# pennucci/PulsePortraiture

Measured on AMD Instinct MI355X. Metric: subint_fits_per_sec, higher is better.
Workload: dtype f64

## Files before the change

pulseportraiture_amd/csrc/pp_common.h:

```cpp
#pragma once
#include <hip/hip_runtime.h>
#include <stdint.h>
#include <type_traits>

namespace pp {

#define PP_DCONST 4149.377593360996
#define PP_TWO_PI 6.283185307179586476925286766559
#define PP_LN10 2.302585092994045684017991454684

typedef double2 cplx;

__device__ __forceinline__ cplx cmul(cplx a, cplx b) {
    return make_double2(fma(a.x, b.x, -a.y * b.y), fma(a.x, b.y, a.y * b.x));
}
__device__ __forceinline__ cplx cmulc(cplx a, cplx b) {
    return make_double2(fma(a.x, b.x, a.y * b.y), fma(a.y, b.x, -a.x * b.y));
}
__device__ __forceinline__ cplx cadd(cplx a, cplx b) { return make_double2(a.x + b.x, a.y + b.y); }
__device__ __forceinline__ cplx csub(cplx a, cplx b) { return make_double2(a.x - b.x, a.y - b.y); }
__device__ __forceinline__ cplx cmul_mi(cplx a) { return make_double2(a.y, -a.x); }
__device__ __forceinline__ double cnorm(cplx a) { return fma(a.x, a.x, a.y * a.y); }

template <typename T>
__device__ __forceinline__ const T* as_global(const T* p) {
    typedef const T __attribute__((address_space(1)))* gp_t;
    return (const T*)(gp_t)(uintptr_t)p;
}

template <typename T>
__device__ __forceinline__ T load_uniform(const T* p) {
    typedef const T __attribute__((address_space(4)))* cp_t;
    return *(cp_t)(uintptr_t)p;
}

__device__ __forceinline__ double rn_pin(double r) { asm volatile("" : "+v"(r)); return r; }
__device__ __forceinline__ double mul_rn(double a, double b) { return rn_pin(a * b); }
__device__ __forceinline__ double add_rn(double a, double b) { return rn_pin(a + b); }
__device__ __forceinline__ double sub_rn(double a, double b) { return rn_pin(a - b); }

__device__ __forceinline__ double recip_ge1(double x) {
    double y = __builtin_amdgcn_rcp(x);
    y = fma(fma(-x, y, 1.0), y, y);
    y = fma(fma(-x, y, 1.0), y, y);
    return (x < 1e300) ? y : 0.0;
}

template <bool SC>
__device__ __forceinline__ double kconst(double v) {
    if (SC) asm volatile("" : "+s"(v));
    return v;
}
template <bool SC = false>
__device__ __forceinline__ void sincos_turns(double t, double* sn, double* cs) {
    const double q = rint(4.0 * t);
    const double y = fma(-0.25, q, t);
    const double u = y * y;
    double ps = kconst<SC>(0x1.aaec32af93359p-4);
    ps = fma(ps, u, kconst<SC>(-0x1.6fadb9f155744p-1));
    ps = fma(ps, u, kconst<SC>(0x1.e8f434d018d63p+1));
    ps = fma(ps, u, kconst<SC>(-0x1.e3074fde8871fp+3));
    ps = fma(ps, u, kconst<SC>(0x1.50783487ee782p+5));
    ps = fma(ps, u, kconst<SC>(-0x1.32d2cce62bd86p+6));
    ps = fma(ps, u, kconst<SC>(0x1.466bc6775aae2p+6));
    ps = fma(ps, u, kconst<SC>(-0x1.4abbce625be53p+5));
    ps = fma(ps, u, kconst<SC>(0x1.921fb54442d18p+2));
    const double s0 = ps * y;
    double pc = kconst<SC>(0x1.20c62c2f2d7f5p-2);
    pc = fma(pc, u, kconst<SC>(-0x1.b6e24f44b128fp+0));
    pc = fma(pc, u, kconst<SC>(0x1.f9d38a3763cc3p+2));
    pc = fma(pc, u, kconst<SC>(-0x1.a6d1f2a204a8cp+4));
    pc = fma(pc, u, kconst<SC>(0x1.e1f506891babbp+5));
    pc = fma(pc, u, kconst<SC>(-0x1.55d3c7e3cbffap+6));
    pc = fma(pc, u, kconst<SC>(0x1.03c1f081b5ac4p+6));
    pc = fma(pc, u, kconst<SC>(-0x1.3bd3cc9be45dep+4));
    const double c0 = fma(pc, u, 1.0);
    const int qi = (int)q;
    const bool odd = qi & 1;
    const double so = odd ? c0 : s0, co = odd ? s0 : c0;
    *sn = (qi & 2) ? -so : so;
    *cs = ((qi + 1) & 2) ? -co : co;
}

template <bool SC = false>
__device__ __forceinline__ cplx unit_phasor(double k, double phi) {
    double pfrac = phi - rint(phi);
    double prod = k * pfrac;
    double err = fma(k, pfrac, -prod);
    double r = (prod - rint(prod)) + err;
    double s, c;
    sincos_turns<SC>(r, &s, &c);
    return make_double2(c, s);
}

template <int W>
__device__ __forceinline__ double group_sum(double v) {
#pragma unroll
    for (int o = W / 2; o > 0; o >>= 1) v += __shfl_xor(v, o, 64);
    return v;
}
template <int W>
__device__ __forceinline__ double group_max(double v) {
#pragma unroll
    for (int o = W / 2; o > 0; o >>= 1) v = fmax(v, __shfl_xor(v, o, 64));
    return v;
}

__device__ __forceinline__ int wave_reduce16_index(int lane) { return (lane >> 2) & 15; }
template <int NS>
__device__ __forceinline__ double wave_reduce16(const double (&s)[NS], int lane) {
    double t8[8], t4[4], t2[2];
    const bool b5 = lane & 32, b4 = lane & 16, b3 = lane & 8, b2 = lane & 4;
#pragma unroll
    for (int j = 0; j < 8; ++j) {
        const double hi = (j + 8 < NS) ? s[j + 8] : 0.0;
        const double keep = b5 ? hi : s[j], send = b5 ? s[j] : hi;
        t8[j] = keep + __shfl_xor(send, 32, 64);
    }
#pragma unroll
    for (int j = 0; j < 4; ++j) {
        const double keep = b4 ? t8[j + 4] : t8[j], send = b4 ? t8[j] : t8[j + 4];
        t4[j] = keep + __shfl_xor(send, 16, 64);
    }
#pragma unroll
    for (int j = 0; j < 2; ++j) {
        const double keep = b3 ? t4[j + 2] : t4[j], send = b3 ? t4[j] : t4[j + 2];
        t2[j] = keep + __shfl_xor(send, 8, 64);
    }
    const double keep = b2 ? t2[1] : t2[0], send = b2 ? t2[0] : t2[1];
    double v = keep + __shfl_xor(send, 4, 64);
    v += __shfl_xor(v, 2, 64);
    v += __shfl_xor(v, 1, 64);
    return v;
}

template <int NS>
__device__ __forceinline__ double wave_reduce_lds(const double (&s)[NS], int lane, double* buf) {
    static_assert(NS <= 16, "one value per lane quad");
    const int wpos = (lane >> 4) * 17 + (lane & 15);
#pragma unroll
    for (int q = 0; q < NS; ++q) buf[q * 68 + wpos] = s[q];
    const int q = min(lane >> 2, NS - 1), part = lane & 3;
    const double* src = buf + q * 68 + part * 17;
    double v = 0.0;
#pragma unroll
    for (int t = 0; t < 16; ++t) v += src[t];
    v += __shfl_xor(v, 1, 64);
    v += __shfl_xor(v, 2, 64);
    return v;
}
#define PP_WRED_DOUBLES(NS) ((NS) * 68)

template <int NV>
__device__ inline void block_sum(double (&v)[NV], double* scratch) {
    const int lane = threadIdx.x & 63, wid = threadIdx.x >> 6, nw = blockDim.x >> 6;
#pragma unroll
    for (int i = 0; i < NV; ++i) v[i] = group_sum<64>(v[i]);
    __syncthreads();
    if (lane == 0) {
#pragma unroll
        for (int i = 0; i < NV; ++i) scratch[wid * NV + i] = v[i];
    }
    __syncthreads();
#pragma unroll
    for (int i = 0; i < NV; ++i) {
        double s = 0.0;
        for (int w = 0; w < nw; ++w) s += scratch[w * NV + i];
        v[i] = s;
    }
}

template <int NV, int C0>
__device__ __forceinline__ void wave_totals_to(const double (&v)[NV], int lane, double* dst) {
    constexpr int n = (NV - C0) < 16 ? (NV - C0) : 16;
    double part[n];
#pragma unroll
    for (int j = 0; j < n; ++j) part[j] = v[C0 + j];
    const double tot = wave_reduce16<n>(part, lane);
    if ((lane & 3) == 0 && (lane >> 2) < n) dst[C0 + (lane >> 2)] = tot;
    if constexpr (C0 + 16 < NV) wave_totals_to<NV, C0 + 16>(v, lane, dst);
}
#define PP_BSUM_DOUBLES(NW, NVMAX) (2 * (NW) * ((NVMAX) + 1))
template <int NV, int NVMAX>
__device__ __forceinline__ void block_sum_t(double (&v)[NV], double* scratch, int& flip, double* mx = nullptr) {
    static_assert(NV <= NVMAX, "scratch sized for NVMAX values");
    const int lane = threadIdx.x & 63, wid = threadIdx.x >> 6, nw = blockDim.x >> 6;
    double* buf = scratch + flip * nw * (NVMAX + 1);
    flip ^= 1;
    wave_totals_to<NV, 0>(v, lane, buf + wid * (NV + 1));
    if (mx) {
        const double m = group_max<64>(*mx);
        if (lane == 0) buf[wid * (NV + 1) + NV] = m;
    }
    __syncthreads();
#pragma unroll
    for (int i = 0; i < NV; ++i) {
        double s = 0.0;
        for (int w = 0; w < nw; ++w) s += buf[w * (NV + 1) + i];
        v[i] = s;
    }
    if (mx) {
        double m = buf[NV];
        for (int w = 1; w < nw; ++w) m = fmax(m, buf[w * (NV + 1) + NV]);
        *mx = m;
    }
}

struct SubState {
    double x[5];
    double xe[5];
    double f;
    double g[5];
    double H[25];
    double f0, g0[5], H0[25];
    double radius;
    double pred_red;
    int hits_boundary;
    int iter, nfev, status, done, cur;
    int npass;
    double xl[5], fl, gl[5], Hl[25];
    int fresh;
    int recentred;
    int nmodel;
    int model;
    double xprev[5];
    double geo[4];
};

#define PP_NACC 21
constexpr int PP_CHUNK_CHANNELS = 256;
#define PP_NCS 9
#define PP_TJ 10
#define PP_TSTRIDE (PP_TJ + 2)
#define PP_TAY_PAIR_STRIDE 2
__device__ __forceinline__ size_t tay_idx(size_t row, int q) { return row * PP_TSTRIDE + (size_t)q; }

}
```

pulseportraiture_amd/csrc/pp_fftq.h:

```cpp
#pragma once
#include "pp_fft.h"

namespace pp {

__device__ __forceinline__ void lane_swap32(double& a, double& b) {
    unsigned alo = (unsigned)__double2loint(a), ahi = (unsigned)__double2hiint(a);
    unsigned blo = (unsigned)__double2loint(b), bhi = (unsigned)__double2hiint(b);
    auto r0 = __builtin_amdgcn_permlane32_swap(alo, blo, false, false);
    auto r1 = __builtin_amdgcn_permlane32_swap(ahi, bhi, false, false);
    a = __hiloint2double((int)r1[0], (int)r0[0]);
    b = __hiloint2double((int)r1[1], (int)r0[1]);
}
__device__ __forceinline__ void lane_swap16(double& a, double& b) {
    unsigned alo = (unsigned)__double2loint(a), ahi = (unsigned)__double2hiint(a);
    unsigned blo = (unsigned)__double2loint(b), bhi = (unsigned)__double2hiint(b);
    auto r0 = __builtin_amdgcn_permlane16_swap(alo, blo, false, false);
    auto r1 = __builtin_amdgcn_permlane16_swap(ahi, bhi, false, false);
    a = __hiloint2double((int)r1[0], (int)r0[0]);
    b = __hiloint2double((int)r1[1], (int)r0[1]);
}

__device__ __forceinline__ int fftq_lambda(int t) { return 4 * (t >> 4) + (t & 3) + 16 * ((t >> 2) & 3); }
__device__ __forceinline__ int fftq_lane_of(int lam) { return 16 * ((lam >> 2) & 3) + (lam & 3) + 4 * ((lam >> 4) & 3); }

constexpr int FFTQ_LDS_ELEMS = 4 * 272;

template <int WHEN = 0, typename T1, typename T2, typename Mid>
__device__ __forceinline__ void fftq1024_from(cplx (&v)[16], cplx* lds, T1 get_t1, T2 get_t2, int tid,
                                              double* power, Mid mid) {
    dft16_first(v);
    if (WHEN == 0) mid();
    const cplx t1 = get_t1();
    dft16_second(v);
    {
        cplx wq[16];
        wq[1] = t1;
#pragma unroll
        for (int j = 2; j < 16; ++j) {
            if (j % 2 == 0) {
                const cplx h = wq[j / 2];
                wq[j] = make_double2(fma(h.x, h.x, -h.y * h.y), 2.0 * h.x * h.y);
            } else wq[j] = cmul(wq[j - 1], wq[1]);
        }
#pragma unroll
        for (int j = 1; j < 16; ++j) v[j] = cmul(v[j], wq[j]);
    }
    if (WHEN == 1) mid();
    const cplx t2 = get_t2();
#pragma unroll
    for (int j = 0; j < 8; ++j) {
        lane_swap32(v[j].x, v[j + 8].x);
        lane_swap32(v[j].y, v[j + 8].y);
    }
#pragma unroll
    for (int j = 0; j < 16; ++j) {
        if (j & 4) continue;
        lane_swap16(v[j].x, v[j + 4].x);
        lane_swap16(v[j].y, v[j + 4].y);
    }
    if (WHEN == 2) mid();
    dft16_first(v);
    {
        const cplx w2 = make_double2(fma(t2.x, t2.x, -t2.y * t2.y), 2.0 * t2.x * t2.y);
        const cplx w3 = cmul(w2, t2);
#pragma unroll
        for (int c = 0; c < 4; ++c) {
            v[4 + c] = cmul(v[4 + c], t2);
            v[8 + c] = cmul(v[8 + c], w2);
            v[12 + c] = cmul(v[12 + c], w3);
        }
    }
    {
        cplx* wbase = lds + (tid >> 4) * 272 + 17 * (tid & 15);
#pragma unroll
        for (int j = 0; j < 16; ++j) wbase[j] = v[j];
        lds_sync<64>();
        const cplx* rbase = lds + (tid >> 4) * 272 + (tid & 15);
#pragma unroll
        for (int j = 0; j < 16; ++j) v[j] = rbase[17 * j];
        lds_sync<64>();
    }
    if (WHEN == 3) mid();
    dft_reg<16>(v);
    if (power) {
        double acc = 0.0;
#pragma unroll
        for (int j = 0; j < 16; ++j) {
            if (j == 0 && tid == 0) { const double dM = v[0].x - v[0].y; acc += dM * dM; }
            else acc += cnorm(v[j]);
        }
        *power += acc;
    }
}

template <int WHEN = 0, typename Mid>
__device__ __forceinline__ void fftq1024(cplx (&v)[16], cplx* lds, const cplx t1, const cplx t2, int tid,
                                         double* power, Mid mid) {
    fftq1024_from<WHEN>(v, lds, [&]() { return t1; }, [&]() { return t2; }, tid, power, mid);
}

__device__ __forceinline__ int fftq512_lambda(int t) {
    return 4 * ((t >> 5) & 1) + 2 * ((t >> 4) & 1) + 32 * ((t >> 3) & 1) + 16 * ((t >> 2) & 1) + 8 * ((t >> 1) & 1) + (t & 1);
}
__device__ __forceinline__ int fftq512_lane_of(int lam) {
    return 32 * ((lam >> 2) & 1) + 16 * ((lam >> 1) & 1) + 8 * ((lam >> 5) & 1) + 4 * ((lam >> 4) & 1) + 2 * ((lam >> 3) & 1) + (lam & 1);
}
constexpr int FFTQ512_LDS_ELEMS = 8 * 72;

__device__ __forceinline__ double lane_xor8(double v) {
    int lo = __double2loint(v), hi = __double2hiint(v);
    lo = __builtin_amdgcn_update_dpp(lo, lo, 0x128, 0xF, 0xF, false);
    hi = __builtin_amdgcn_update_dpp(hi, hi, 0x128, 0xF, 0xF, false);
    return __hiloint2double(hi, lo);
}

template <int WHEN = 0, typename Mid>
__device__ __forceinline__ void fftq512(cplx (&v)[8], cplx* lds, const cplx t1, const cplx t2, const cplx t3, int tid,
                                        double* power, Mid mid) {
    dft_reg<8>(v);
    if (WHEN == 0) mid();
    {
        cplx wq[8];
        wq[1] = t1;
#pragma unroll
        for (int j = 2; j < 8; ++j) {
            if (j % 2 == 0) {
                const cplx h = wq[j / 2];
                wq[j] = make_double2(fma(h.x, h.x, -h.y * h.y), 2.0 * h.x * h.y);
            } else wq[j] = cmul(wq[j - 1], wq[1]);
        }
#pragma unroll
        for (int j = 1; j < 8; ++j) v[j] = cmul(v[j], wq[j]);
    }
#pragma unroll
    for (int j = 0; j < 4; ++j) {
        lane_swap32(v[j].x, v[j + 4].x);
        lane_swap32(v[j].y, v[j + 4].y);
    }
#pragma unroll
    for (int j = 0; j < 8; ++j) {
        if (j & 2) continue;
        lane_swap16(v[j].x, v[j + 2].x);
        lane_swap16(v[j].y, v[j + 2].y);
    }
    dft4(v[0], v[2], v[4], v[6]);
    dft4(v[1], v[3], v[5], v[7]);
    {
        const cplx w2 = make_double2(fma(t2.x, t2.x, -t2.y * t2.y), 2.0 * t2.x * t2.y);
        const cplx w3 = cmul(w2, t2);
#pragma unroll
        for (int c = 0; c < 2; ++c) {
            v[2 + c] = cmul(v[2 + c], t2);
            v[4 + c] = cmul(v[4 + c], w2);
            v[6 + c] = cmul(v[6 + c], w3);
        }
    }
    {
        const bool up = (tid & 8) != 0;
        const double sg = up ? -1.0 : 1.0;
        const cplx w = up ? t3 : make_double2(1.0, 0.0);
#pragma unroll
        for (int j = 0; j < 8; ++j) {
            const cplx p = make_double2(lane_xor8(v[j].x), lane_xor8(v[j].y));
            const cplx d = make_double2(fma(sg, v[j].x, p.x), fma(sg, v[j].y, p.y));
            v[j] = cmul(d, w);
        }
    }
    {
        cplx* wbase = lds + (tid >> 3) * 72 + 9 * (tid & 7);
#pragma unroll
        for (int j = 0; j < 8; ++j) wbase[j] = v[j];
        lds_sync<64>();
        const cplx* rbase = lds + (tid >> 3) * 72 + (tid & 7);
#pragma unroll
        for (int j = 0; j < 8; ++j) v[j] = rbase[9 * j];
        lds_sync<64>();
    }
    if (WHEN == 3) mid();
    dft_reg<8>(v);
    if (power) {
        double acc = 0.0;
#pragma unroll
        for (int j = 0; j < 8; ++j) {
            if (j == 0 && tid == 0) { const double dM = v[0].x - v[0].y; acc += dM * dM; }
            else acc += cnorm(v[j]);
        }
        *power += acc;
    }
}

template <int M> struct FftQ;
template <> struct FftQ<1024> {
    static constexpr int R = 16, LDS_ELEMS = FFTQ_LDS_ELEMS;
    static __device__ __forceinline__ int lambda(int t) { return fftq_lambda(t); }
    static __device__ __forceinline__ int lane_of(int lam) { return fftq_lane_of(lam); }
    template <int WHEN, typename Mid>
    static __device__ __forceinline__ void run(cplx (&v)[16], cplx* lds, const cplx* twB, int tid, double* power, Mid mid) {
        const cplx t1 = twB[2 * tid], t2 = twB[32 * (tid & 15)];
        fftq1024<WHEN>(v, lds, t1, t2, tid, power, mid);
    }
};
template <> struct FftQ<512> {
    static constexpr int R = 8, LDS_ELEMS = FFTQ512_LDS_ELEMS;
    static __device__ __forceinline__ int lambda(int t) { return fftq512_lambda(t); }
    static __device__ __forceinline__ int lane_of(int lam) { return fftq512_lane_of(lam); }
    template <int WHEN, typename Mid>
    static __device__ __forceinline__ void run(cplx (&v)[8], cplx* lds, const cplx* twB, int tid, double* power, Mid mid) {
        const cplx t1 = twB[2 * tid], t2 = twB[16 * (tid & 15)], t3 = twB[64 * (tid & 7)];
        fftq512<WHEN>(v, lds, t1, t2, t3, tid, power, mid);
    }
};


__device__ __forceinline__ cplx split_pair(const cplx zk, cplx zc, const cplx wb) {
    zc.y = -zc.y;
    const cplx E = make_double2(zk.x + zc.x, zk.y + zc.y);
    const cplx O = make_double2(zk.x - zc.x, zk.y - zc.y);
    const cplx wo = cmul(wb, O);
    return make_double2(E.x + wo.y, E.y - wo.x);
}

template <int N>
__device__ __forceinline__ void taylor_terms(const bool first, double (&tm)[N], const cplx x, const cplx z, const double kap) {
    static_assert(PP_TJ == 10 && N >= PP_TSTRIDE, "power ladder written for order 10");
    const double p2 = kap * kap, p4 = p2 * p2, p6 = p4 * p2, p8 = p4 * p4, p10 = p8 * p2;
    const double ui = z.y * kap;
    const double ax = fabs(x.x) + fabs(x.y);
    if (first) {
        tm[0] = z.x;
        tm[1] = ui;
        tm[2] = p2 * z.x;
        tm[3] = p2 * ui;
        tm[4] = p4 * z.x;
        tm[5] = p4 * ui;
        tm[6] = p6 * z.x;
        tm[7] = p6 * ui;
        tm[8] = p8 * z.x;
        tm[9] = p8 * ui;
        tm[10] = p10 * z.x;
        tm[11] = (p10 * kap) * ax;
    } else {
        tm[0] += z.x;
        tm[1] += ui;
        tm[2] = fma(p2, z.x, tm[2]);
        tm[3] = fma(p2, ui, tm[3]);
        tm[4] = fma(p4, z.x, tm[4]);
        tm[5] = fma(p4, ui, tm[5]);
        tm[6] = fma(p6, z.x, tm[6]);
        tm[7] = fma(p6, ui, tm[7]);
        tm[8] = fma(p8, z.x, tm[8]);
        tm[9] = fma(p8, ui, tm[9]);
        tm[10] = fma(p10, z.x, tm[10]);
        tm[11] = fma(p10 * kap, ax, tm[11]);
    }
}

template <typename Raw, int R>
__device__ __forceinline__ void load_row_pieces(Raw (&cur)[1][R], const void* nxrow, const int tid, const int k0, const int k1) {
    const char* gb = reinterpret_cast<const char*>(nxrow);
    const unsigned boff = (unsigned)tid * (unsigned)sizeof(Raw);
#pragma unroll
    for (int k = 0; k < R; ++k)
        if (k >= k0 && k < k1) cur[0][k] = load_row_once<Raw>(gb + (size_t)(k * 64) * sizeof(Raw) + boff);
}

}
```

pulseportraiture_amd/csrc/pp_xspec1024q.h:

```cpp
#pragma once
#include "pp_fftq.h"


namespace pp {

constexpr unsigned PP_TICKET_WINDOW_NUM = 3u, PP_TICKET_WINDOW_DEN = 4u;
__device__ __forceinline__ int ticket_moment(const long long nrows) {
    const unsigned share = (unsigned)(nrows / (long long)gridDim.x) + 1u;
    return 1 + (int)(((blockIdx.x * 2654435761u) >> 8) % (share * PP_TICKET_WINDOW_NUM / PP_TICKET_WINDOW_DEN + 1u));
}

template <int M, typename Tin>
__device__ __forceinline__ const Tin* next_row_of(const XspecArgs& a, const unsigned more_nx, const int i_nx, const int n_nx,
                                                  const size_t rc) {
    const size_t rn = more_nx ? (size_t)sub_of(a.act, i_nx) * a.nchan_full + (a.coff + n_nx * a.cstep) : rc;
    return reinterpret_cast<const Tin*>(a.data) + rn * (2 * M);
}

constexpr int FFTQ_FREE_ELEM0 = 3 * 272 + 16, FFTQ_FREE_PITCH = 17;

template <int M, bool TAIL, bool ONE = true>
__device__ __forceinline__ void store_row_results(const XspecArgs& a, const size_t rc, const int tid, double tv) {
    constexpr int H = M + 1, kc = (int)(0.75 * H);
  if constexpr (ONE) {
    const int q = wave_reduce16_index(tid);
    const double th = 0.5 * tv;
    double val = (q <= PP_TJ && ((q & 3) == 1 || (q & 3) == 2)) ? -th : th;
    double* dst = a.tay + tay_idx(rc, q < PP_TSTRIDE ? q : 0);
    if (q >= PP_TSTRIDE) { val = tv; dst = a.sdraw + rc; }
    if (TAIL) {
        const double nz = sqrt(tv / (2.0 * M) / (double)(H - kc));
        if (q > PP_TSTRIDE) { val = nz; dst = a.noise + rc; }
    }
    typedef double __attribute__((address_space(1)))* gdp_t;
    *(gdp_t)(uintptr_t)dst = val;
  } else {
    if ((tid & 3) == 0) {
        const int q = wave_reduce16_index(tid);
        if (q < PP_TSTRIDE) {
            tv *= 0.5;
            a.tay[tay_idx(rc, q)] = (q <= PP_TJ && ((q & 3) == 1 || (q & 3) == 2)) ? -tv : tv;
        }
    }
    if (tid == 4 * PP_TSTRIDE) a.sdraw[rc] = tv;
    if (TAIL && tid == 4 * (PP_TSTRIDE + 1)) a.noise[rc] = sqrt(tv / (2.0 * M) / (double)(H - kc));
  }
}

__device__ __forceinline__ void first_row_landed() { __builtin_amdgcn_s_waitcnt(0x0F70); }

constexpr int Q_PREFETCH_F64 = 1, Q_PREFETCH_F32 = 0;
template <typename Tin, bool TAIL>
__global__ __launch_bounds__(64, 2) void k_xspec_q1024(XspecArgs a) {
    constexpr int M = 1024, T = 64, R1 = 16, PER1 = 1;
    constexpr int NSL = 7;
    typedef typename RawOf<Tin>::type Raw;
    constexpr int NRED = PP_TSTRIDE + (TAIL ? 2 : 1);
    static_assert(NRED <= 16, "wave_reduce_lds takes 16 values");
    constexpr int WRED = PP_WRED_DOUBLES(NRED) / 2;
    constexpr int LDSN = WRED > FFTQ_LDS_ELEMS ? WRED : FFTQ_LDS_ELEMS;
    static_assert(2 * LDSN >= PP_TAIL_LDS_DOUBLES, "tail_work's layout of this kernel's LDS");
    constexpr bool F64 = sizeof(Tin) == 8;
    constexpr int NML = (F64 && TAIL) ? 2 : 0;
    constexpr bool TWL = F64 && !TAIL, TWR = F64 && TAIL;
    constexpr bool ROWTOP = !TAIL;
    constexpr int NTW = TWL ? 2 : 0;
    __shared__ cplx lds[LDSN + 64 * (NML + NTW)];
    static_assert(sizeof(lds) <= 19456, "eight workgroups per CU");
    static_assert(FFTQ_FREE_ELEM0 + 15 * FFTQ_FREE_PITCH < FFTQ_LDS_ELEMS && FFTQ_FREE_ELEM0 >= 64 * (TAIL ? 12 : 7) &&
                  2 * FFTQ_FREE_ELEM0 >= PP_WRED_DOUBLES(NRED), "t2's elements are outside everything a row writes");
    cplx* const ldsm = lds + LDSN + threadIdx.x;
    int tid = threadIdx.x;
    const long long nrows = (long long)a.nsub * a.nchan;
    Raw cur[PER1][R1];
    cplx t1 = a.twB[2 * tid], t2 = a.twB[32 * (tid & 15)];
    const int lam0 = fftq_lambda(tid);
    cplx wb0 = a.twB[lam0 ? lam0 : 64];
    const cplx wbT = a.twB[64];
    cplx* const ldt2 = lds + FFTQ_FREE_ELEM0;
    cplx* const ldtw = lds + LDSN + 64 * NML;
    auto put_lane_consts = [&](const cplx p1, const cplx p2, const cplx pb) {
        if (!TWL) return;
        ldt2[FFTQ_FREE_PITCH * (tid & 15)] = p2;
        ldtw[tid] = p1;
        ldtw[64 + tid] = pb;
        lds_sync<T>();
    };
    put_lane_consts(t1, t2, wb0);
    int tail_after = 0x7fffffff;
    if (a.tail) tail_after = ticket_moment(nrows);
    RowWalk<true> rw;
    rw.start(nrows, a.mwords, a.ticket, a.ticket_base);
    long long row = rw.row;
    int n = 0, i = 0;
    if (rw.more) {
        n = __builtin_amdgcn_readfirstlane((int)(row / a.nsub));
        i = __builtin_amdgcn_readfirstlane((int)(row % a.nsub));
        const size_t rc = (size_t)sub_of(a.act, i) * a.nchan_full + (a.coff + n * a.cstep);
        stage_load_global<M, T, R1>(cur, reinterpret_cast<const Tin*>(a.data) + rc * (2 * M), tid);
    }
    cplx mv2[NSL];
    const cplx* mheld = nullptr;
    const cplx* mrow = nullptr;
    int n_held = -1, ktn = 0;
    int i_nx = i, n_nx = n;
    if (ROWTOP) first_row_landed();
#pragma unroll 1
    for (int phase = 0; phase < 2; ++phase) {
    if (phase == 1) {
        if (!a.tail) break;
        tail_work(a.tail, reinterpret_cast<double*>(lds), 2 * (LDSN + 64 * NML), tid, 1);
        tail_after = 0x7fffffff;
        if (TWL) {
            const int lamr = fftq_lambda(tid);
            put_lane_consts(as_global(a.twB)[2 * tid], as_global(a.twB)[32 * (tid & 15)], as_global(a.twB)[lamr ? lamr : 64]);
        }
    }
    for (; rw.more && tail_after != 0; rw.advance(), row = rw.row, i = i_nx, n = n_nx, --tail_after) {
        rw.draw(a.ticket);
        rw.peek(nrows, a.ticket_base, a.mwords);
        asm volatile("" : "+v"(tid));
        const int lam = fftq_lambda(tid);
        const bool l0 = (lam == 0);
        const int kb = l0 ? 64 : lam;
        if (TWR) {
            t1 = as_global(a.twB)[2 * tid];
            t2 = as_global(a.twB)[32 * (tid & 15)];
            wb0 = as_global(a.twB)[kb];
        } else if (!TWL) {
            asm volatile("" : "+v"(t1.x), "+v"(t1.y), "+v"(t2.x), "+v"(t2.y), "+v"(wb0.x), "+v"(wb0.y));
        }
        const int ia = sub_of(a.act, i), ne = a.coff + n * a.cstep;
        const size_t rc = (size_t)ia * a.nchan_full + ne;
        if (channel_lookup(a, ia, n, ne, M, n_held, mrow, ktn) && mrow != mheld) {
#pragma unroll
            for (int j = 0; j < NSL; ++j) {
                const cplx mval = mrow[kb + 64 * j - 1];
                if (j < NSL - NML) mv2[j] = mval; else ldsm[64 * (j - (NSL - NML))] = mval;
            }
            mheld = mrow;
        }
        const double phin = ROWTOP ? load_uniform(a.ph0 + rc) : a.ph0[rc];
        double sd = 0.0;
        cplx v[R1];
#pragma unroll
        for (int k = 0; k < R1; ++k) v[k] = to_cplx(cur[0][k]);
        constexpr bool HALVES = F64;
        const Tin* nxrow = nullptr;
        auto load_some = [&](int k0, int k1) { load_row_pieces<Raw>(cur, nxrow, tid, k0, k1); };
        rw.next(i, n, i_nx, n_nx, nrows, a.nsub, a.ticket_base, a.ticket, a.mwords);
        nxrow = next_row_of<M, Tin>(a, rw.more_nx, i_nx, n_nx, rc);
        auto prefetch = [&]() {
            __builtin_amdgcn_sched_barrier(0);
            load_some(0, HALVES ? R1 / 2 : R1);
            __builtin_amdgcn_sched_barrier(0);
        };
        fftq1024_from<(sizeof(Tin) == 8 ? Q_PREFETCH_F64 : Q_PREFETCH_F32)>(
            v, lds, [&]() { return NTW ? ldtw[tid] : t1; }, [&]() { return TWL ? ldt2[FFTQ_FREE_PITCH * (tid & 15)] : t2; },
            tid, &sd, prefetch);
        __builtin_amdgcn_sched_barrier(0);
        {
            cplx* pub = lds + tid;
#pragma unroll
            for (int r = 0; r < NSL; ++r) pub[64 * r] = v[9 + r];
            if (TAIL) {
#pragma unroll
                for (int r = 0; r < 5; ++r) pub[64 * (NSL + r)] = v[r];
            }
            lds_sync<T>();
        }
        if (NTW) wb0 = ldtw[64 + tid];
        double tail = 0.0;
        if (TAIL) {
            const double h = 0.70710678118654752440;
            const cplx* pt = lds + fftq_lane_of((64 - lam) & 63) + (l0 ? 64 : 0);
            cplx wt = l0 ? make_double2(-h, -h) : cmul(wb0, make_double2(-h, -h));
#pragma unroll
            for (int kd = 12; kd < 16; ++kd) {
                tail += cnorm(split_pair(v[kd], pt[64 * (NSL + 15 - kd)], wt));
                wt = cmul(wt, wbT);
            }
            tail *= 0.25;
            if (tid == 0) { const double dM = v[0].x - v[0].y; tail += dM * dM; }
        }
        if (HALVES) {
            __builtin_amdgcn_sched_barrier(0);
            load_some(R1 / 2, R1);
            __builtin_amdgcn_sched_barrier(0);
        }
        const cplx* pc = lds + fftq_lane_of((64 - lam) & 63);
        const cplx el = unit_phasor<true>((double)kb, phin);
        const cplx wst = make_double2(bcast_lane0(el.x), bcast_lane0(el.y));
        cplx e = el, wb = wb0;
        const int ktu = __builtin_amdgcn_readfirstlane(ktn);
        const double kap0 = PP_TWO_PI * (double)kb;
        double tm[PP_TSTRIDE];
        cplx zc_nx = pc[64 * 6];
#pragma unroll
        for (int j = 0; j < NSL; ++j) {
            if (j > 0 && !(64 * j < ktu)) break;
            const cplx zc = zc_nx;
            if (j + 1 < NSL && 64 * (j + 1) < ktu) zc_nx = pc[64 * (5 - j)];
            if (j == 0 || 64 * j < ktu) {
                const cplx dd = split_pair(csel(l0, v[j + 1], v[j]), zc, wb);
                const cplx mj = (j < NSL - NML) ? mv2[j < NSL - NML ? j : 0] : ldsm[64 * (j - (NSL - NML))];
                const cplx x = cmulc(dd, mj);
                const cplx z = cmul(x, e);
                const double kap = j == 0 ? kap0 : kap0 + kconst<true>(PP_TWO_PI * (double)(64 * j));
                taylor_terms(j == 0, tm, x, z, kap);
            }
            if (j + 1 < NSL && 64 * (j + 1) < ktu) {
                wb = cmul(wb, wbT);
                e = cmul(e, wst);
            }
        }
        double tr[NRED];
#pragma unroll
        for (int j = 0; j < PP_TSTRIDE; ++j) tr[j] = tm[j];
        tr[PP_TSTRIDE] = sd;
        if (TAIL) tr[NRED - 1] = tail;
        lds_sync<T>();
        double tv = wave_reduce_lds(tr, tid, reinterpret_cast<double*>(lds));
        store_row_results<M, TAIL, ROWTOP>(a, rc, tid, tv);
        lds_sync<T>();
    }
    }
    if (a.tail) tail_work(a.tail, reinterpret_cast<double*>(lds), 2 * (LDSN + 64 * NML), tid, 1 << 30);
}


constexpr int PP_QF512_WPS = 3;
template <int M, typename Tin, bool TAIL>
__global__ __launch_bounds__(64, (M == 1024 ? 2 : PP_QF512_WPS)) void k_xspec_qf(XspecArgs a) {
    typedef FftQ<M> Q;
    constexpr int T = 64, R1 = Q::R, PER1 = 1;
    constexpr int NSL = R1;
    constexpr int JT = (3 * NSL) / 4;
    static_assert((int)(0.75 * (M + 1)) == 64 * JT, "the noise tail starts on a slot boundary");
    typedef typename RawOf<Tin>::type Raw;
    constexpr int NRED = PP_TSTRIDE + (TAIL ? 2 : 1);
    constexpr int WRED = PP_WRED_DOUBLES(NRED) / 2;
    constexpr int LDSN0 = Q::LDS_ELEMS > 64 * NSL ? Q::LDS_ELEMS : 64 * NSL;
    constexpr int LDSN = WRED > LDSN0 ? WRED : LDSN0;
    static_assert(M != 1024 || 2 * LDSN >= PP_TAIL_LDS_DOUBLES, "tail_work's layout of this kernel's LDS");
    __shared__ cplx lds[LDSN];
    int tid = threadIdx.x;
    constexpr bool QTOP = M == 1024 && !TAIL;
    const long long nrows = (long long)a.nsub * a.nchan;
    Raw cur[PER1][R1];
    const cplx wbT = a.twB[64];
    int tail_after = 0x7fffffff;
    if (M == 1024 && a.tail) tail_after = ticket_moment(nrows);
    RowWalk<true> rw;
    rw.start(nrows, a.mwords, a.ticket, a.ticket_base);
    long long row = rw.row;
    int n = 0, i = 0;
    if (rw.more) {
        n = __builtin_amdgcn_readfirstlane((int)(row / a.nsub));
        i = __builtin_amdgcn_readfirstlane((int)(row % a.nsub));
        const size_t rc = (size_t)sub_of(a.act, i) * a.nchan_full + (a.coff + n * a.cstep);
        stage_load_global<M, T, R1>(cur, reinterpret_cast<const Tin*>(a.data) + rc * (2 * M), tid);
    }
    int i_nx = i, n_nx = n;
    const cplx* mrow = nullptr;
    int n_held = -1, ktn = 0;
    constexpr bool MHOLD = M == 512;
    cplx mv[NSL];
    const cplx* mheld = nullptr;
    if (QTOP) first_row_landed();
#pragma unroll 1
    for (int phase = 0; phase < 2; ++phase) {
    if (phase == 1) {
        if (!(M == 1024 && a.tail)) break;
        tail_work(a.tail, reinterpret_cast<double*>(lds), 2 * LDSN, tid, 1);
        tail_after = 0x7fffffff;
    }
    for (; rw.more && tail_after != 0; rw.advance(), row = rw.row, i = i_nx, n = n_nx, --tail_after) {
        rw.draw(a.ticket);
        rw.peek(nrows, a.ticket_base, a.mwords);
        asm volatile("" : "+v"(tid));
        const int lam = Q::lambda(tid);
        const bool l0 = (lam == 0);
        const int kb = l0 ? 64 : lam;
        const cplx wb0 = as_global(a.twB)[kb];
        const int ia = sub_of(a.act, i), ne = a.coff + n * a.cstep;
        const size_t rc = (size_t)ia * a.nchan_full + ne;
        const bool looked = channel_lookup(a, ia, n, ne, M, n_held, mrow, ktn);
        if (MHOLD && looked && mrow != mheld) {
#pragma unroll
            for (int j = 0; j < NSL; ++j) mv[j] = mrow[kb + 64 * j - 1];
            mheld = mrow;
        }
        const double phin = QTOP ? load_uniform(a.ph0 + rc) : a.ph0[rc];
        double sd = 0.0;
        cplx v[R1];
#pragma unroll
        for (int k = 0; k < R1; ++k) v[k] = to_cplx(cur[0][k]);
        auto template_loads = [&]() {
            if (MHOLD) return;
            __builtin_amdgcn_sched_barrier(0);
#pragma unroll
            for (int j = 0; j < NSL; ++j) mv[j] = mrow[kb + 64 * j - 1];
            __builtin_amdgcn_sched_barrier(0);
        };
        Q::template run<3>(v, lds, as_global(a.twB), tid, &sd, template_loads);
        __builtin_amdgcn_sched_barrier(0);
        {
            cplx* pub = lds + tid;
#pragma unroll
            for (int s = 0; s < NSL; ++s) pub[64 * s] = v[s];
            lds_sync<T>();
        }
        const Tin* nxrow;
        auto load_some = [&](int k0, int k1) { load_row_pieces<Raw>(cur, nxrow, tid, k0, k1); };
        {
            __builtin_amdgcn_sched_barrier(0);
            rw.next(i, n, i_nx, n_nx, nrows, a.nsub, a.ticket_base, a.ticket, a.mwords);
            nxrow = next_row_of<M, Tin>(a, rw.more_nx, i_nx, n_nx, rc);
            load_some(0, R1 / 2);
            __builtin_amdgcn_sched_barrier(0);
        }
        const cplx* pc = lds + Q::lane_of((64 - lam) & 63);
        const cplx el = unit_phasor<true>((double)kb, phin);
        const cplx wst = make_double2(bcast_lane0(el.x), bcast_lane0(el.y));
        cplx e = el, wb = wb0;
        const int ktu = __builtin_amdgcn_readfirstlane(ktn);
        const double kap0 = PP_TWO_PI * (double)kb;
        double tm[PP_TSTRIDE];
        double tail = 0.0;
        cplx zc_nx = pc[64 * (NSL - 1)];
#pragma unroll
        for (int j = 0; j < NSL; ++j) {
            if (!TAIL && j > NSL / 2 && !(64 * j < ktu)) break;
            const cplx zc = zc_nx;
            if (j + 1 < NSL && (TAIL || 64 * (j + 1) < ktu)) zc_nx = pc[64 * (NSL - 2 - j)];
            if (j == NSL / 2) {
                __builtin_amdgcn_sched_barrier(0);
                load_some(R1 / 2, R1);
                __builtin_amdgcn_sched_barrier(0);
            }
            const bool keep = (j == 0 || 64 * j < ktu);
            if (keep || (TAIL && j >= JT - 1)) {
                const cplx dd = split_pair(csel(l0, v[(j + 1) & (NSL - 1)], v[j]), zc, wb);
                if (TAIL && j >= JT - 1) {
                    const double pw = cnorm(dd);
                    tail += (j >= JT || l0) ? pw : 0.0;
                }
              if (keep) {
                const cplx x = cmulc(dd, mv[j]);
                const cplx z = cmul(x, e);
                const double kap = j == 0 ? kap0 : kap0 + kconst<true>(PP_TWO_PI * (double)(64 * j));
                taylor_terms(j == 0, tm, x, z, kap);
              }
            }
            if (TAIL || (j + 1 < NSL && 64 * (j + 1) < ktu)) {
                wb = cmul(wb, wbT);
                e = cmul(e, wst);
            }
        }
        double tr[NRED];
#pragma unroll
        for (int j = 0; j < PP_TSTRIDE; ++j) tr[j] = tm[j];
        tr[PP_TSTRIDE] = sd;
        if (TAIL) tr[NRED - 1] = 0.25 * tail;
        lds_sync<T>();
        double tv = wave_reduce_lds(tr, tid, reinterpret_cast<double*>(lds));
        store_row_results<M, TAIL, QTOP>(a, rc, tid, tv);
        lds_sync<T>();
    }
    }
    if (M == 1024 && a.tail) tail_work(a.tail, reinterpret_cast<double*>(lds), 2 * LDSN, tid, 1 << 30);
}

}
```

Measured before the change: 74580.

## Overlap row epilogue reduction with next row setup and hide phasor work in transpose

Splits the per-row LDS wave reduction into a publish step and a finish step. The finish runs after the next row's setup (ticket draw, channel lookup, phase load), so that global-load latency overlaps the LDS reads. The FFT's mid transpose is interleaved with the twiddle multiplies, and the unit-phasor computation is scheduled inside the transpose's LDS wait window. The quad reduction uses DPP moves instead of shuffles. This adds restructured control flow and more live registers, which may hurt occupancy or scheduling.

```diff
diff --git a/pulseportraiture_amd/csrc/pp_common.h b/pulseportraiture_amd/csrc/pp_common.h
--- a/pulseportraiture_amd/csrc/pp_common.h
+++ b/pulseportraiture_amd/csrc/pp_common.h
@@ -135,19 +135,45 @@
 }
 
 template <int NS>
-__device__ __forceinline__ double wave_reduce_lds(const double (&s)[NS], int lane, double* buf) {
+__device__ __forceinline__ void wave_reduce_lds_publish(const double (&s)[NS], int lane, double* buf) {
     static_assert(NS <= 16, "one value per lane quad");
     const int wpos = (lane >> 4) * 17 + (lane & 15);
 #pragma unroll
     for (int q = 0; q < NS; ++q) buf[q * 68 + wpos] = s[q];
+}
+template <int CTRL>
+__device__ __forceinline__ double quad_perm(double v) {
+    int lo = __double2loint(v), hi = __double2hiint(v);
+    lo = __builtin_amdgcn_mov_dpp(lo, CTRL, 0xF, 0xF, true);
+    hi = __builtin_amdgcn_mov_dpp(hi, CTRL, 0xF, 0xF, true);
+    return __hiloint2double(hi, lo);
+}
+template <int NS, bool ALL_FIRST = false>
+__device__ __forceinline__ double wave_reduce_lds_finish(int lane, const double* buf) {
     const int q = min(lane >> 2, NS - 1), part = lane & 3;
     const double* src = buf + q * 68 + part * 17;
     double v = 0.0;
+    if (ALL_FIRST) {
+        double x[16];
+#pragma unroll
+        for (int t = 0; t < 16; ++t) x[t] = src[t];
+        __builtin_amdgcn_sched_barrier(0);
+#pragma unroll
+        for (int t = 0; t < 16; ++t) v += x[t];
+        v += quad_perm<0xB1>(v);
+        v += quad_perm<0x4E>(v);
+        return v;
+    }
 #pragma unroll
     for (int t = 0; t < 16; ++t) v += src[t];
     v += __shfl_xor(v, 1, 64);
     v += __shfl_xor(v, 2, 64);
     return v;
+}
+template <int NS>
+__device__ __forceinline__ double wave_reduce_lds(const double (&s)[NS], int lane, double* buf) {
+    wave_reduce_lds_publish(s, lane, buf);
+    return wave_reduce_lds_finish<NS>(lane, buf);
 }
 #define PP_WRED_DOUBLES(NS) ((NS) * 68)
 
diff --git a/pulseportraiture_amd/csrc/pp_fftq.h b/pulseportraiture_amd/csrc/pp_fftq.h
--- a/pulseportraiture_amd/csrc/pp_fftq.h
+++ b/pulseportraiture_amd/csrc/pp_fftq.h
@@ -25,9 +25,10 @@
 
 constexpr int FFTQ_LDS_ELEMS = 4 * 272;
 
-template <int WHEN = 0, typename T1, typename T2, typename Mid>
+template <int WHEN = 0, typename T1, typename T2, typename Mid, typename Shadow = NoMid>
 __device__ __forceinline__ void fftq1024_from(cplx (&v)[16], cplx* lds, T1 get_t1, T2 get_t2, int tid,
-                                              double* power, Mid mid) {
+                                              double* power, Mid mid, Shadow shadow = Shadow()) {
+    constexpr bool PIECES = !IsNoMid<Shadow>::value;
     dft16_first(v);
     if (WHEN == 0) mid();
     const cplx t1 = get_t1();
@@ -60,7 +61,11 @@
     }
     if (WHEN == 2) mid();
     dft16_first(v);
-    {
+    if (PIECES) {
+        cplx* wbase = lds + (tid >> 4) * 272 + 17 * (tid & 15);
+        __builtin_amdgcn_sched_barrier(0);
+#pragma unroll
+        for (int c = 0; c < 4; ++c) wbase[c] = v[c];
         const cplx w2 = make_double2(fma(t2.x, t2.x, -t2.y * t2.y), 2.0 * t2.x * t2.y);
         const cplx w3 = cmul(w2, t2);
 #pragma unroll
@@ -68,6 +73,32 @@
             v[4 + c] = cmul(v[4 + c], t2);
             v[8 + c] = cmul(v[8 + c], w2);
             v[12 + c] = cmul(v[12 + c], w3);
+            __builtin_amdgcn_sched_barrier(0);
+            wbase[4 + c] = v[4 + c];
+            wbase[8 + c] = v[8 + c];
+            wbase[12 + c] = v[12 + c];
+            __builtin_amdgcn_sched_barrier(0);
+        }
+        lds_sync<64>();
+        const cplx* rbase = lds + (tid >> 4) * 272 + (tid & 15);
+#pragma unroll
+        for (int q = 0; q < 4; ++q) {
+#pragma unroll
+            for (int m = 0; m < 4; ++m) v[4 * m + q] = rbase[17 * (4 * m + q)];
+            __builtin_amdgcn_sched_barrier(0);
+        }
+        shadow();
+        __builtin_amdgcn_sched_barrier(0);
+        lds_sync<64>();
+    } else {
+    {
+        const cplx w2 = make_double2(fma(t2.x, t2.x, -t2.y * t2.y), 2.0 * t2.x * t2.y);
+        const cplx w3 = cmul(w2, t2);
+#pragma unroll
+        for (int c = 0; c < 4; ++c) {
+            v[4 + c] = cmul(v[4 + c], t2);
+            v[8 + c] = cmul(v[8 + c], w2);
+            v[12 + c] = cmul(v[12 + c], w3);
         }
     }
     {
@@ -79,6 +110,7 @@
 #pragma unroll
         for (int j = 0; j < 16; ++j) v[j] = rbase[17 * j];
         lds_sync<64>();
+    }
     }
     if (WHEN == 3) mid();
     dft_reg<16>(v);
diff --git a/pulseportraiture_amd/csrc/pp_xspec1024q.h b/pulseportraiture_amd/csrc/pp_xspec1024q.h
--- a/pulseportraiture_amd/csrc/pp_xspec1024q.h
+++ b/pulseportraiture_amd/csrc/pp_xspec1024q.h
@@ -104,7 +104,45 @@
     const cplx* mrow = nullptr;
     int n_held = -1, ktn = 0;
     int i_nx = i, n_nx = n;
-    if (ROWTOP) first_row_landed();
+    constexpr bool EPI_SPLIT = !TAIL, XPOSE_SHADOW = !TAIL;
+    size_t rc = 0, rc_done = 0;
+    const Tin* nxrow = nullptr;
+    double phin = 0.0;
+    auto row_top = [&]() {
+        rw.draw(a.ticket);
+        rw.peek(nrows, a.ticket_base, a.mwords);
+        asm volatile("" : "+v"(tid));
+        const int lamt = fftq_lambda(tid);
+        const int kb = lamt ? lamt : 64;
+        if (TWR) {
+            t1 = as_global(a.twB)[2 * tid];
+            t2 = as_global(a.twB)[32 * (tid & 15)];
+            wb0 = as_global(a.twB)[kb];
+        } else if (!TWL) {
+            asm volatile("" : "+v"(t1.x), "+v"(t1.y), "+v"(t2.x), "+v"(t2.y), "+v"(wb0.x), "+v"(wb0.y));
+        }
+        const int ia = sub_of(a.act, i), ne = a.coff + n * a.cstep;
+        rc = (size_t)ia * a.nchan_full + ne;
+        if (channel_lookup(a, ia, n, ne, M, n_held, mrow, ktn) && mrow != mheld) {
+#pragma unroll
+            for (int j = 0; j < NSL; ++j) {
+                const cplx mval = mrow[kb + 64 * j - 1];
+                if (j < NSL - NML) mv2[j] = mval; else ldsm[64 * (j - (NSL - NML))] = mval;
+            }
+            mheld = mrow;
+        }
+        phin = ROWTOP ? load_uniform(a.ph0 + rc) : a.ph0[rc];
+        rw.next(i, n, i_nx, n_nx, nrows, a.nsub, a.ticket_base, a.ticket, a.mwords);
+        nxrow = next_row_of<M, Tin>(a, rw.more_nx, i_nx, n_nx, rc);
+    };
+    auto finish_row = [&](const size_t rcp) {
+        __builtin_amdgcn_sched_barrier(0);
+        const double tv = wave_reduce_lds_finish<NRED, true>(tid, reinterpret_cast<const double*>(lds));
+        store_row_results<M, TAIL, ROWTOP>(a, rcp, tid, tv);
+        lds_sync<T>();
+        __builtin_amdgcn_sched_barrier(0);
+    };
+    if (ROWTOP && !EPI_SPLIT) first_row_landed();
 #pragma unroll 1
     for (int phase = 0; phase < 2; ++phase) {
     if (phase == 1) {
@@ -116,49 +154,42 @@
             put_lane_consts(as_global(a.twB)[2 * tid], as_global(a.twB)[32 * (tid & 15)], as_global(a.twB)[lamr ? lamr : 64]);
         }
     }
-    for (; rw.more && tail_after != 0; rw.advance(), row = rw.row, i = i_nx, n = n_nx, --tail_after) {
-        rw.draw(a.ticket);
-        rw.peek(nrows, a.ticket_base, a.mwords);
-        asm volatile("" : "+v"(tid));
+    if constexpr (EPI_SPLIT) {
+        if (!(rw.more && tail_after != 0)) continue;
+        row_top();
+        if (ROWTOP) first_row_landed();
+    }
+    for (;;) {
+        if constexpr (!EPI_SPLIT) {
+            if (!(rw.more && tail_after != 0)) break;
+            row_top();
+        }
+        double sd = 0.0;
+        cplx v[R1];
+#pragma unroll
+        for (int k = 0; k < R1; ++k) v[k] = to_cplx(cur[0][k]);
+        constexpr bool HALVES = F64;
+        auto load_some = [&](int k0, int k1) { load_row_pieces<Raw>(cur, nxrow, tid, k0, k1); };
+        auto prefetch = [&]() {
+            __builtin_amdgcn_sched_barrier(0);
+            load_some(0, HALVES ? R1 / 2 : R1);
+            __builtin_amdgcn_sched_barrier(0);
+        };
+        cplx el, wst;
+        auto phasors = [&]() {
+            const int lamp = fftq_lambda(tid);
+            el = unit_phasor<true>((double)(lamp ? lamp : 64), phin);
+            wst = make_double2(bcast_lane0(el.x), bcast_lane0(el.y));
+        };
+        auto get_t1 = [&]() { return NTW ? ldtw[tid] : t1; };
+        auto get_t2 = [&]() { return TWL ? ldt2[FFTQ_FREE_PITCH * (tid & 15)] : t2; };
+        constexpr int WHEN = sizeof(Tin) == 8 ? Q_PREFETCH_F64 : Q_PREFETCH_F32;
+        if constexpr (XPOSE_SHADOW) fftq1024_from<WHEN>(v, lds, get_t1, get_t2, tid, &sd, prefetch, phasors);
+        else fftq1024_from<WHEN>(v, lds, get_t1, get_t2, tid, &sd, prefetch);
+        __builtin_amdgcn_sched_barrier(0);
         const int lam = fftq_lambda(tid);
         const bool l0 = (lam == 0);
         const int kb = l0 ? 64 : lam;
-        if (TWR) {
-            t1 = as_global(a.twB)[2 * tid];
-            t2 = as_global(a.twB)[32 * (tid & 15)];
-            wb0 = as_global(a.twB)[kb];
-        } else if (!TWL) {
-            asm volatile("" : "+v"(t1.x), "+v"(t1.y), "+v"(t2.x), "+v"(t2.y), "+v"(wb0.x), "+v"(wb0.y));
-        }
-        const int ia = sub_of(a.act, i), ne = a.coff + n * a.cstep;
-        const size_t rc = (size_t)ia * a.nchan_full + ne;
-        if (channel_lookup(a, ia, n, ne, M, n_held, mrow, ktn) && mrow != mheld) {
-#pragma unroll
-            for (int j = 0; j < NSL; ++j) {
-                const cplx mval = mrow[kb + 64 * j - 1];
-                if (j < NSL - NML) mv2[j] = mval; else ldsm[64 * (j - (NSL - NML))] = mval;
-            }
-            mheld = mrow;
-        }
-        const double phin = ROWTOP ? load_uniform(a.ph0 + rc) : a.ph0[rc];
-        double sd = 0.0;
-        cplx v[R1];
-#pragma unroll
-        for (int k = 0; k < R1; ++k) v[k] = to_cplx(cur[0][k]);
-        constexpr bool HALVES = F64;
-        const Tin* nxrow = nullptr;
-        auto load_some = [&](int k0, int k1) { load_row_pieces<Raw>(cur, nxrow, tid, k0, k1); };
-        rw.next(i, n, i_nx, n_nx, nrows, a.nsub, a.ticket_base, a.ticket, a.mwords);
-        nxrow = next_row_of<M, Tin>(a, rw.more_nx, i_nx, n_nx, rc);
-        auto prefetch = [&]() {
-            __builtin_amdgcn_sched_barrier(0);
-            load_some(0, HALVES ? R1 / 2 : R1);
-            __builtin_amdgcn_sched_barrier(0);
-        };
-        fftq1024_from<(sizeof(Tin) == 8 ? Q_PREFETCH_F64 : Q_PREFETCH_F32)>(
-            v, lds, [&]() { return NTW ? ldtw[tid] : t1; }, [&]() { return TWL ? ldt2[FFTQ_FREE_PITCH * (tid & 15)] : t2; },
-            tid, &sd, prefetch);
-        __builtin_amdgcn_sched_barrier(0);
         {
             cplx* pub = lds + tid;
 #pragma unroll
@@ -189,8 +220,7 @@
             __builtin_amdgcn_sched_barrier(0);
         }
         const cplx* pc = lds + fftq_lane_of((64 - lam) & 63);
-        const cplx el = unit_phasor<true>((double)kb, phin);
-        const cplx wst = make_double2(bcast_lane0(el.x), bcast_lane0(el.y));
+        if (!XPOSE_SHADOW) phasors();
         cplx e = el, wb = wb0;
         const int ktu = __builtin_amdgcn_readfirstlane(ktn);
         const double kap0 = PP_TWO_PI * (double)kb;
@@ -220,9 +250,21 @@
         tr[PP_TSTRIDE] = sd;
         if (TAIL) tr[NRED - 1] = tail;
         lds_sync<T>();
-        double tv = wave_reduce_lds(tr, tid, reinterpret_cast<double*>(lds));
-        store_row_results<M, TAIL, ROWTOP>(a, rc, tid, tv);
-        lds_sync<T>();
+        if constexpr (!EPI_SPLIT) {
+            double tv = wave_reduce_lds(tr, tid, reinterpret_cast<double*>(lds));
+            store_row_results<M, TAIL, ROWTOP>(a, rc, tid, tv);
+            lds_sync<T>();
+            rw.advance(), row = rw.row, i = i_nx, n = n_nx, --tail_after;
+        } else {
+            wave_reduce_lds_publish(tr, tid, reinterpret_cast<double*>(lds));
+            lds_sync<T>();
+            rc_done = rc;
+            rw.advance(), row = rw.row, i = i_nx, n = n_nx, --tail_after;
+            const bool go_on = rw.more && tail_after != 0;
+            if (go_on) row_top();
+            finish_row(rc_done);
+            if (!go_on) break;
+        }
     }
     }
     if (a.tail) tail_work(a.tail, reinterpret_cast<double*>(lds), 2 * (LDSN + 64 * NML), tid, 1 << 30);
```

Measured after the change: 75320, median of 6. About the same (+1.0%).
